# g8a9/multi-modal-emotion

Hardware: AMD Instinct MI355X
Metric: utterances/sec fwd+bwd (+clip_grad_norm_+AdamW inside the timed step), TAV (BERT+Wav2Vec2+VideoMAE) b=32, 1/2/4/8 MI355X (higher is better)
Workload: dtype bf16; 1 GPU; tav_nn.py TAV preset B (bert 12 L + wav2vec2 12 L / 768 + videomae 12 L / 768 on 16 frames + fusion 12 L), global batch 32 = 32 per GPU x 1, text 128 tok, audio 80000 samples, video 16x3x224x224 (104 fusion / 1464 encoder tokens), 547.0 GFLOP forward per utterance; global_batch=32, per_gpu_batch=32, parallelism=dp1, weights=random init (seeded), no checkpoints offline, launch=hipGraph replay

## Files before the change

### include/tavhip.h

```cpp
#ifndef TAVHIP_H
#define TAVHIP_H
#include <stdint.h>

#ifdef __cplusplus
extern "C" {
#endif

enum { TAV_F32 = 0, TAV_BF16 = 1, TAV_FP8 = 2 ,
       TAV_U8 = 3 ,
       TAV_I16 = 4  };
enum {
    TAV_ERR_NULL = -1,
    TAV_ERR_SHAPE = -2,
    TAV_ERR_DTYPE = -3,
    TAV_ERR_ALIGN = -4,
    TAV_ERR_NO_RCCL = -5
};

int tav_version(void);
const char* tav_error_string(int code);

typedef struct tav_gemm_nt_args {
    const void* A; const void* B; void* C;
    void* C_pre;
// ... 15 lines not shown
} tav_gemm_nt_args;
int tav_gemm_nt(const tav_gemm_nt_args* args, void* stream);
int tav_gemm_nt_schedule(const tav_gemm_nt_args* args, int32_t* tile, int32_t* rows_first, int32_t* tile_rest);

typedef struct tav_gemm_tn_args {
    const void* A; const void* B;
    float* slabs;
    float* out;
    float* dbias;
    float* bias_partials;
    int64_t N1, N2;
    int64_t lda, ldb;
    int64_t rows_per_batch, nbatch;
    int64_t a_zb, b_zb;
    int32_t chunk_rows, nsplit;
    int32_t perm_inner, perm_outer;
    int32_t dtype;
    int32_t accumulate;
    float scale;
} tav_gemm_tn_args;
int tav_gemm_tn_splits(int64_t n1, int64_t n2, int64_t rows_per_batch, int64_t nbatch, int32_t* chunk_rows, int32_t* nsplit);
int tav_gemm_tn(const tav_gemm_tn_args* args, void* stream);

typedef struct tav_gemm_tn_problem {
    const void* A; const void* B;
    float* out;
    float* dbias;
    int64_t N1, N2, lda, ldb;
} tav_gemm_tn_problem;
int tav_gemm_tn_grouped(const tav_gemm_tn_problem* problems, int32_t nproblems, int64_t rows, int32_t dtype, void* stream);
int64_t tav_gemm_tn_grouped_ws_bytes(const tav_gemm_tn_problem* problems, int32_t nproblems, int64_t rows, int32_t dtype, int32_t flags);
int tav_gemm_tn_grouped_ws(const tav_gemm_tn_problem* problems, int32_t nproblems, int64_t rows, int32_t dtype, void* workspace,
                           int64_t workspace_bytes, int32_t flags, void* stream);

int tav_fp8_amax_partials(int64_t rows, int64_t cols);
int tav_fp8_amax(const void* x, int32_t dtype, int64_t rows, int64_t cols, int64_t ld, float* partials, float* scales, void* stream);
int tav_fp8_quantize(const void* x, int32_t dtype, int64_t rows, int64_t cols, int64_t ld, const float* scales, void* q, int64_t ld_q, void* qt,
                     int64_t ld_qt, int64_t rows_pad, void* stream);
int tav_fp8_quantize_delayed(const void* x, int32_t dtype, int64_t rows, int64_t cols, int64_t ld, float* state, void* q, int64_t ld_q, void* qt,
                             int64_t ld_qt, int64_t rows_pad, void* stream);
int tav_fp8_roll_states(float* states, int64_t n, void* stream);
int tav_splitk_reduce(const float* slabs, float* out, int32_t nsplit, int64_t n_elems, int32_t accumulate, void* stream);

int tav_colsum(const void* x, int32_t dtype, int64_t M, int64_t N, int64_t ld, float* partials, int32_t nparts, float* out,
               int32_t accumulate, void* stream);

typedef struct tav_attn_args {
    const void* q; const void* k; const void* v;
    void* o;
    const float* key_mask;
    float* lse;
    float* corr;
    void* o_soft;
    const void* dout; void* dq; void* dk; void* dv;
    float* delta;
    int64_t B, S, nheads;
    int64_t ld_q, ld_k, ld_v, ld_o, ld_do, ld_dq, ld_dk, ld_dv;
    int32_t dtype, mask_mode;
    float scale;
    int32_t q_prescaled;
} tav_attn_args;
int tav_attn_fwd(const tav_attn_args* args, void* stream);
int tav_attn_bwd(const tav_attn_args* args, void* stream);
int tav_attn_fwd_len(const tav_attn_args* args, const int32_t* seq_lens, void* stream);
int tav_attn_bwd_len(const tav_attn_args* args, const int32_t* seq_lens, void* stream);
int tav_attn_probs(const tav_attn_args* args, float* probs, const float* head_scale, int64_t hs_bstride, void* stream);
// ... 190 lines not shown
```

### multi-modal-emotion_amd/_lib.py

```python
import ctypes as C
import os

import torch

_HERE = os.path.dirname(os.path.abspath(__file__))
LIB_PATH = os.environ.get("TAV_LIB") or os.path.join(_HERE, "libtavhip.so")

TAV_F32, TAV_BF16, TAV_FP8, TAV_U8, TAV_I16 = 0, 1, 2, 3, 4
ABI_VERSION = 7

i32, i64, f32, vp = C.c_int32, C.c_int64, C.c_float, C.c_void_p


class GemmNTArgs(C.Structure):
    _fields_ = [("A", vp), ("B", vp), ("C", vp), ("C_pre", vp), ("bias", vp), ("gelu_in", vp), ("resid", vp),
                ("M", i64), ("N", i64), ("K", i64),
                ("lda", i64), ("ldb", i64), ("ldc", i64), ("ld_pre", i64), ("ld_gelu_in", i64), ("ld_resid", i64),
                ("nzb", i32), ("nzg", i32),
                ("a_zb", i64), ("a_zg", i64), ("b_zb", i64), ("b_zg", i64), ("c_zb", i64), ("c_zg", i64), ("bias_zg", i64),
                ("in_dtype", i32), ("out_dtype", i32), ("act", i32), ("accumulate", i32), ("alpha", f32),
                ("a_dequant", vp), ("b_dequant", vp), ("gelu_zb", i64), ("tile_m_hint", i32)]


class GemmTNArgs(C.Structure):
    _fields_ = [("A", vp), ("B", vp), ("slabs", vp), ("out", vp), ("dbias", vp), ("bias_partials", vp),
                ("N1", i64), ("N2", i64), ("lda", i64), ("ldb", i64), ("rows_per_batch", i64), ("nbatch", i64),
                ("a_zb", i64), ("b_zb", i64), ("chunk_rows", i32), ("nsplit", i32), ("perm_inner", i32), ("perm_outer", i32),
                ("dtype", i32), ("accumulate", i32), ("scale", f32)]


class GemmTNProblem(C.Structure):
    _fields_ = [("A", vp), ("B", vp), ("out", vp), ("dbias", vp), ("N1", i64), ("N2", i64), ("lda", i64), ("ldb", i64)]


class AttnArgs(C.Structure):
    _fields_ = [("q", vp), ("k", vp), ("v", vp), ("o", vp), ("key_mask", vp), ("lse", vp), ("corr", vp), ("o_soft", vp),
                ("dout", vp), ("dq", vp), ("dk", vp), ("dv", vp), ("delta", vp),
                ("B", i64), ("S", i64), ("nheads", i64),
                ("ld_q", i64), ("ld_k", i64), ("ld_v", i64), ("ld_o", i64), ("ld_do", i64), ("ld_dq", i64), ("ld_dk", i64), ("ld_dv", i64),
                ("dtype", i32), ("mask_mode", i32), ("scale", f32), ("q_prescaled", i32)]


class LnArgs(C.Structure):
    _fields_ = [("x", vp), ("x_dtype", i32), ("gamma", vp), ("beta", vp), ("y_f32", vp), ("y_lp", vp), ("lp_dtype", i32),
                ("mean", vp), ("rstd", vp),
                ("dy", vp), ("dy_dtype", i32), ("dx_add", vp), ("dx_f32", vp), ("dx_lp", vp),
                ("dgamma", vp), ("dbeta", vp), ("partials", vp), ("accumulate_params", i32),
                ("rows", i64), ("W", i64), ("ld_x", i64), ("ld_y", i64), ("ld_dy", i64), ("ld_dx", i64), ("eps", f32), ("act", i32),
                ("defer_param_reduce", i32)]


class LnReduceItem(C.Structure):
    _fields_ = [("partials", vp), ("dgamma", vp), ("dbeta", vp), ("nblocks", i32), ("W", i32), ("accumulate", i32), ("pad_", i32)]


LN_REDUCE_MAX = 64


class TextEmbedArgs(C.Structure):
    _fields_ = [("ids", vp), ("word", vp), ("pos", vp), ("type", vp), ("gamma", vp), ("beta", vp), ("pre", vp), ("pos_ids", vp),
                ("y_f32", vp), ("y_lp", vp), ("lp_dtype", i32), ("mean", vp), ("rstd", vp),
                ("B", i64), ("S", i64), ("W", i64), ("vocab", i64), ("max_pos", i64), ("pad_id", i32), ("eps", f32)]


class ClipXform(C.Structure):
    _fields_ = [("src_dtype", i32), ("T", i32), ("H", i32), ("W", i32), ("sT", i64), ("sH", i64), ("sW", i64), ("sC", i64),
                ("nf", i32), ("frame", i32 * 32), ("crop_top", i32), ("crop_left", i32), ("crop_h", i32), ("crop_w", i32),
                ("mid_h", i32), ("mid_w", i32), ("out_h", i32), ("out_w", i32), ("hflip", i32), ("vflip", i32),
                ("scale", f32 * 3), ("shift", f32 * 3)]


class ResampleArgs(C.Structure):
    _fields_ = [("src_dtype", i32), ("C", i32), ("L", i64), ("sC", i64), ("sL", i64), ("o", i32), ("n", i32), ("width", i32), ("ntap", i32),
                ("first_max", i32), ("reserved", i32), ("T_row", i64)]


_SIGS = {
    "tav_version": (C.c_int, []),
    "tav_error_string": (C.c_char_p, [C.c_int]),
    "tav_gemm_nt": (C.c_int, [C.POINTER(GemmNTArgs), vp]),
    "tav_gemm_nt_schedule": (C.c_int, [C.POINTER(GemmNTArgs), C.POINTER(i32), C.POINTER(i32), C.POINTER(i32)]),
    "tav_gemm_tn_splits": (C.c_int, [i64, i64, i64, i64, C.POINTER(i32), C.POINTER(i32)]),
    "tav_gemm_tn": (C.c_int, [C.POINTER(GemmTNArgs), vp]),
    "tav_gemm_tn_grouped": (C.c_int, [C.POINTER(GemmTNProblem), i32, i64, i32, vp]),
    "tav_gemm_tn_grouped_ws_bytes": (C.c_int64, [C.POINTER(GemmTNProblem), i32, i64, i32, i32]),
    "tav_gemm_tn_grouped_ws": (C.c_int, [C.POINTER(GemmTNProblem), i32, i64, i32, vp, i64, i32, vp]),
    "tav_colsum": (C.c_int, [vp, i32, i64, i64, i64, vp, i32, vp, i32, vp]),
    "tav_fp8_amax_partials": (C.c_int, [i64, i64]),
    "tav_fp8_amax": (C.c_int, [vp, i32, i64, i64, i64, vp, vp, vp]),
    "tav_fp8_quantize": (C.c_int, [vp, i32, i64, i64, i64, vp, vp, i64, vp, i64, i64, vp]),
    "tav_fp8_quantize_delayed": (C.c_int, [vp, i32, i64, i64, i64, vp, vp, i64, vp, i64, i64, vp]),
    "tav_fp8_roll_states": (C.c_int, [vp, i64, vp]),
    "tav_splitk_reduce": (C.c_int, [vp, vp, i32, i64, i32, vp]),
    "tav_comm_rccl_version": (C.c_int, [C.POINTER(i32)]),
    "tav_comm_unique_id": (C.c_int, [vp]),
    "tav_comm_init_rank": (C.c_int, [C.POINTER(vp), i32, vp, i32]),
    "tav_comm_destroy": (C.c_int, [vp]),
    "tav_allreduce_bucket": (C.c_int, [vp, i64, i32, vp, vp]),
    "tav_attn_fwd": (C.c_int, [C.POINTER(AttnArgs), vp]),
    "tav_attn_bwd": (C.c_int, [C.POINTER(AttnArgs), vp]),
    "tav_attn_fwd_len": (C.c_int, [C.POINTER(AttnArgs), vp, vp]),
    "tav_attn_bwd_len": (C.c_int, [C.POINTER(AttnArgs), vp, vp]),
    "tav_attn_probs": (C.c_int, [C.POINTER(AttnArgs), vp, vp, i64, vp]),
    "tav_head_scale": (C.c_int, [vp, vp, vp, i32, vp, i64, f32, i64, i64, i64, i64, i64, i64, vp]),
    "tav_ln_fwd": (C.c_int, [C.POINTER(LnArgs), vp]),
    "tav_ln_bwd": (C.c_int, [C.POINTER(LnArgs), vp]),
    "tav_ln_bwd_partials": (C.c_int, [i64]),
    "tav_ln_param_reduce_multi": (C.c_int, [C.POINTER(LnReduceItem), i32, vp]),
    "tav_cast_weight": (C.c_int, [vp, i64, i64, vp, i64, vp, i64, i32, vp]),
    "tav_cast_weights_multi": (C.c_int, [vp, i32, i32, vp]),
    "tav_cast_conv_weight": (C.c_int, [vp, i64, i64, i64, vp, vp, vp, i64, i32, vp]),
    "tav_zero_pad_rows": (C.c_int, [vp, i32, i64, i64, i64, i64, vp]),
    "tav_cast2d": (C.c_int, [vp, i32, i64, vp, i32, i64, i64, i64, vp]),
    "tav_transpose2d": (C.c_int, [vp, vp, i32, i64, i64, i64, vp]),
    "tav_add_f32": (C.c_int, [vp, vp, vp, vp, i32, i64, vp]),
    "tav_fill_f32": (C.c_int, [vp, f32, i64, vp]),
    "tav_embed_add_fwd": (C.c_int, [vp, vp, vp, vp, i64, i64, i64, vp]),
    "tav_embed_add_bwd": (C.c_int, [vp, vp, vp, vp, i64, i64, i64, i32, vp]),
    "tav_embed_add_bwd_parts": (C.c_int, [i64]),
# ... 100 lines not shown
```

### multi-modal-emotion_amd/csrc/gemm.hip

```cpp
#include "common.h"
#include <type_traits>
#include "tavhip_internal.h"
#include "gemm_plan.h"

namespace tav {

struct GemmNT {
    const char* A; const char* B; char* C; char* Cpre; const float* bias; const char* gelu_in; const float* resid;
    int M, N, K;
    long lda, ldb, ldc, ld_pre, ld_gelu, ld_resid;
    int nzg;
    long a_zb, a_zg, b_zb, b_zg, c_zb, c_zg, bias_zg;
    long g_zb;
    int act, accumulate;
    float alpha;
    int tiles_m, tiles_n;
    const float* sa; const float* sb;
};

TAV_DEV int swz(int row, int chunk) { return chunk ^ ((row >> 1) & 7); }

enum { NT_GEN = 0, NT_PLAIN = 1, NT_RESID = 2, NT_GELU_D = 3, NT_MUL_D = 4 };
template <typename T, typename TO, int TM, int NST, int NW, int TNW, int EPI = NT_GEN>
__global__ __launch_bounds__(64 * NW, NW == 4 ? 2 : 1) __attribute__((amdgpu_waves_per_eu(2, 2))) void gemm_nt_kernel(const GemmNT p) {
// ... 503 lines not shown
    for (int a = 0; a < 4; ++a) {
        const int n1 = n1_0 + w1 * 64 + a * 16 + i;
        if (n1 >= p.N1) continue;
#pragma unroll
        for (int b = 0; b < 4; ++b) {
            const int n2 = n2_0 + w2 * 64 + b * 16 + 4 * g;
            if (n2 >= p.N2) continue;
            st4(S + (long)n1 * p.N2 + n2, acc[a][b]);
        }
    }
}

template <typename T>
__global__ __launch_bounds__(256, 2) void gemm_tn_kernel(const GemmTN p) {
    gemm_tn_body<T>(p, xcd_remap(blockIdx.x, p.tiles_1 * p.tiles_2), blockIdx.y);
}

constexpr int TN_GROUP_MAX = 4;
struct GemmTNGroup {
    GemmTN p[TN_GROUP_MAX];
    int tile_end[TN_GROUP_MAX];
    int n;
};
template <typename T>
__global__ __launch_bounds__(256, 2) void gemm_tn_grouped_kernel(const GemmTNGroup grp) {
    const int t = xcd_remap(blockIdx.x, grp.tile_end[grp.n - 1]);
    int g = 0;
#pragma unroll
    for (int k = 0; k < TN_GROUP_MAX - 1; ++k) g += (k < grp.n - 1 && t >= grp.tile_end[k]) ? 1 : 0;
    const int first = g == 0 ? 0 : grp.tile_end[g - 1];
    gemm_tn_body<T>(grp.p[g], t - first, 0);
}

template <typename T>
TAV_DEV void gemm_tn_big_body(const GemmTN& p, const int tile, const int split) {
    using TT = TNTile<T>;
    static_assert(ET<T>::ES == 2, "bf16 only");
    constexpr int ES = 2, KSTEP = ET<T>::KSTEP, KT = 64, ROWB = TT::ROWB;
    constexpr int SUB = KT * ROWB;
    constexpr int STAGE = 4 * SUB;
    extern __shared__ __attribute__((aligned(16))) char smem[];

    const int tid = threadIdx.x, lane = tid & 63, wave = tid >> 6;
    const int g = lane >> 4, i = lane & 15;
    const int w1 = wave >> 1, w2 = wave & 1;

    int t1, t2;
    if (p.tiles_1 >= p.tiles_2) { t1 = tile / p.tiles_2; t2 = tile - t1 * p.tiles_2; }
    else { t2 = tile / p.tiles_1; t1 = tile - t2 * p.tiles_1; }
    const int n1_0 = t1 * 256, n2_0 = t2 * 256;
    const int row_begin = split * p.chunk_rows;
    int row_end = row_begin + p.chunk_rows; row_end = row_end < p.rows_per_batch ? row_end : p.rows_per_batch;
    const int nrows = row_end - row_begin;
    const int nk = nrows > 0 ? (nrows + KT - 1) / KT : 0;

    const int lrow = lane >> 4, lslot = lane & 15;
    const int a_cmax = (p.N1 - n1_0) * ES / 16, b_cmax = (p.N2 - n2_0) * ES / 16;
    const char* Ab0 = p.A + ((long)row_begin * p.lda + n1_0) * ES;
    const char* Bb0 = p.B + ((long)row_begin * p.ldb + n2_0) * ES;
    unsigned offA[2][2], offB[2][2];
#pragma unroll
    for (int h = 0; h < 2; ++h)
#pragma unroll
        for (int j = 0; j < 2; ++j) {
            const int trow = wave * 8 + j * 4 + lrow;
            int ca = 16 * h + TT::sw(trow, lslot); ca = ca < a_cmax ? ca : 0;
// ... 129 lines not shown
    long end4[TN_GROUP_MAX];
    int N1[TN_GROUP_MAX];
    int nbias[TN_GROUP_MAX];
    int n, nsplit;
};
__global__ void tn_group_reduce_kernel(const TNGroupReduce r) {
    const long gid = (long)blockIdx.x * blockDim.x + threadIdx.x;
    if (gid >= r.end4[r.n - 1]) return;
    int k = 0;
#pragma unroll
    for (int q = 0; q < TN_GROUP_MAX - 1; ++q) k += (q < r.n - 1 && gid >= r.end4[q]) ? 1 : 0;
    const long local = gid - (k == 0 ? 0 : r.end4[k - 1]);
    const float* S = r.slabs[k];
    f32x4 v = {0.f, 0.f, 0.f, 0.f};
    for (int s2 = 0; s2 < r.nsplit; ++s2) v += ld4(S + ((long)s2 * r.n4[k] + local) * 4);
    st4(r.out[k] + local * 4, v);
    if (r.dbias[k] && local < r.N1[k]) {
        float b = 0.f;
        for (int s2 = 0; s2 < r.nbias[k]; ++s2) b += r.bias_part[k][(long)s2 * r.N1[k] + local];
        r.dbias[k][local] = b;
    }
}
__global__ void tn_group_bias_reduce_kernel(const TNGroupReduce r, int total_n1) {
    int gid = blockIdx.x * blockDim.x + threadIdx.x;
    if (gid >= total_n1) return;
    int k = 0;
    while (k < r.n - 1 && gid >= r.N1[k]) { gid -= r.N1[k]; ++k; }
    if (!r.dbias[k]) return;
    float b = 0.f;
    for (int s2 = 0; s2 < r.nbias[k]; ++s2) b += r.bias_part[k][(long)s2 * r.N1[k] + gid];
    r.dbias[k][gid] = b;
}

__global__ void splitk_reduce_kernel(const float* __restrict__ S, float* __restrict__ out, int nsplit, long n_elems, int N2,
                                     int inner, int outer, int accumulate, float scale, const float* __restrict__ bias_part,
                                     float* __restrict__ dbias, int N1) {
    const long gid = (long)blockIdx.x * blockDim.x + threadIdx.x;
    if (dbias && gid < N1) {
        float b = 0.f;
        for (int s = 0; s < nsplit; ++s) b += bias_part[(long)s * N1 + gid];
        b *= scale;
        dbias[gid] = accumulate ? dbias[gid] + b : b;
    }
    const long idx4 = gid * 4;
    if (idx4 >= n_elems) return;
    f32x4 v = {0.f, 0.f, 0.f, 0.f};
    for (int s = 0; s < nsplit; ++s) v += ld4(S + (long)s * n_elems + idx4);
    v *= scale;
    if (outer == 1) {
        if (accumulate) v += ld4(out + idx4);
        st4(out + idx4, v);
    } else {
        const long n1 = idx4 / N2; const int n2 = (int)(idx4 - n1 * N2);
#pragma unroll
        for (int e = 0; e < 4; ++e) {
            const int q = n2 + e;
            const long o = n1 * N2 + (long)(q % inner) * outer + q / inner;
            out[o] = accumulate ? out[o] + v[e] : v[e];
        }
    }
}

__global__ void bias_reduce_kernel(const float* __restrict__ part, float* __restrict__ out, int nsplit, int N1, int accumulate, float scale) {
    const int n = blockIdx.x * blockDim.x + threadIdx.x;
    if (n >= N1) return;
    float s = 0.f;
    for (int k = 0; k < nsplit; ++k) s += part[(long)k * N1 + n];
    s *= scale;
    out[n] = accumulate ? out[n] + s : s;
}

template <typename T>
__global__ void colsum_partial_kernel(const T* __restrict__ X, float* __restrict__ part, int M, int N, long ld, int rows_per_block) {
    const int n = blockIdx.x * blockDim.x + threadIdx.x;
    const int r_begin = blockIdx.y * rows_per_block;
    int r_end = r_begin + rows_per_block; r_end = r_end < M ? r_end : M;
    if (n >= N) return;
    float s0 = 0.f, s1 = 0.f, s2 = 0.f, s3 = 0.f;
    int r = r_begin;
    for (; r + 3 < r_end; r += 4) {
        s0 += ET<T>::ld(X + (long)r * ld + n); s1 += ET<T>::ld(X + (long)(r + 1) * ld + n);
        s2 += ET<T>::ld(X + (long)(r + 2) * ld + n); s3 += ET<T>::ld(X + (long)(r + 3) * ld + n);
    }
    for (; r < r_end; ++r) s0 += ET<T>::ld(X + (long)r * ld + n);
    part[(long)blockIdx.y * N + n] = (s0 + s1) + (s2 + s3);
}
__global__ void colsum_final_kernel(const float* __restrict__ part, float* __restrict__ out, int nparts, int N, int accumulate) {
    const int n = blockIdx.x * blockDim.x + threadIdx.x;
    if (n >= N) return;
    float s0 = 0.f, s1 = 0.f, s2 = 0.f, s3 = 0.f;
    int k = 0;
    for (; k + 3 < nparts; k += 4) {
        s0 += part[(long)k * N + n]; s1 += part[(long)(k + 1) * N + n]; s2 += part[(long)(k + 2) * N + n]; s3 += part[(long)(k + 3) * N + n];
// ... 147 lines not shown
    { const int rc = plan::tn_validate_problem(a->A, a->B, a->out, a->N1, a->N2, a->lda, a->ldb, a->a_zb, a->b_zb, a->rows_per_batch, a->nbatch, a->dtype);
      if (rc != 0) return rc; }
    if (a->chunk_rows <= 0 || a->chunk_rows % 64) return TAV_ERR_SHAPE;
    GemmTN p;
    p.A = (const char*)a->A; p.B = (const char*)a->B; p.S = a->slabs;
    p.bias_part = a->dbias ? a->bias_partials : nullptr; p.bias_spread = 0;
    if (a->dbias && !a->bias_partials) return TAV_ERR_NULL;
    p.N1 = (int)a->N1; p.N2 = (int)a->N2; p.lda = a->lda; p.ldb = a->ldb;
    p.rows_per_batch = (int)a->rows_per_batch; p.a_zb = a->a_zb; p.b_zb = a->b_zb;
    p.chunk_rows = a->chunk_rows;
    p.chunks_per_batch = (int)((a->rows_per_batch + a->chunk_rows - 1) / a->chunk_rows);
    const int nsplit = p.chunks_per_batch * (int)a->nbatch;
    if (nsplit != a->nsplit) return TAV_ERR_SHAPE;
    p.tiles_1 = (p.N1 + 127) / 128; p.tiles_2 = (p.N2 + 127) / 128;
    const int inner = a->perm_inner > 0 ? a->perm_inner : p.N2, outer = a->perm_outer > 0 ? a->perm_outer : 1;
    if (outer > 1 && inner * outer != p.N2) return TAV_ERR_SHAPE;
    dim3 grid(p.tiles_1 * p.tiles_2, nsplit), block(256);
    if (a->dtype == TAV_BF16) {
        const size_t lds = 4 * 64 * 256;
        hipLaunchKernelGGL((gemm_tn_kernel<bf16>), grid, block, lds, stream, p);
    } else {
        const size_t lds = 4 * 64 * 512;
        hipLaunchKernelGGL((gemm_tn_kernel<float>), grid, block, lds, stream, p);
    }
    int e = (int)hipGetLastError();
    if (e) return e;
    const long n_elems = (long)p.N1 * p.N2;
    const long nthreads = (n_elems + 3) / 4;
    hipLaunchKernelGGL(splitk_reduce_kernel, dim3((unsigned)((nthreads + 255) / 256)), dim3(256), 0, stream, a->slabs, a->out, nsplit,
                       n_elems, p.N2, inner, outer, a->accumulate, a->scale == 0.f ? 1.f : a->scale, (const float*)a->bias_partials, a->dbias, p.N1);
    return (int)hipGetLastError();
}

extern "C" int tav_colsum(const void* x, int32_t dtype, int64_t M, int64_t N, int64_t ld, float* partials, int32_t nparts, float* out,
                          int32_t accumulate, void* stream_) {
    hipStream_t stream = (hipStream_t)stream_;
    if (!x || !partials || !out) return TAV_ERR_NULL;
    if (M <= 0 || N <= 0 || nparts <= 0) return TAV_ERR_SHAPE;
    const int rows_per_block = (int)((M + nparts - 1) / nparts);
    dim3 grid((unsigned)((N + 255) / 256), nparts), block(256);
    if (dtype == TAV_BF16) hipLaunchKernelGGL((colsum_partial_kernel<bf16>), grid, block, 0, stream, (const bf16*)x, partials, (int)M, (int)N, (long)ld, rows_per_block);
    else if (dtype == TAV_F32) hipLaunchKernelGGL((colsum_partial_kernel<float>), grid, block, 0, stream, (const float*)x, partials, (int)M, (int)N, (long)ld, rows_per_block);
    else return TAV_ERR_DTYPE;
    hipLaunchKernelGGL(colsum_final_kernel, dim3((unsigned)((N + 255) / 256)), dim3(256), 0, stream, partials, out, nparts, (int)N, accumulate);
    return (int)hipGetLastError();
}
```

### multi-modal-emotion_amd/csrc/gemm_plan.h

```cpp
#pragma once
#include <stdint.h>
#include <algorithm>
#include "../../include/tavhip.h"

namespace tav {
namespace plan {

inline int elem_size(int dtype) { return dtype == TAV_FP8 ? 1 : (dtype == TAV_BF16 ? 2 : 4); }

inline int nt_validate(const tav_gemm_nt_args* a, bool need_ptrs) {
    if (!a || (need_ptrs && (!a->A || !a->B || !a->C))) return TAV_ERR_NULL;
    if (a->M <= 0 || a->N <= 0 || a->K <= 0) return TAV_ERR_SHAPE;
    const int es = elem_size(a->in_dtype);
    if (a->in_dtype != TAV_BF16 && a->in_dtype != TAV_F32 && a->in_dtype != TAV_FP8) return TAV_ERR_DTYPE;
    if (a->in_dtype == TAV_F32 && a->out_dtype != TAV_F32) return TAV_ERR_DTYPE;
    if (a->out_dtype != TAV_F32 && a->out_dtype != TAV_BF16) return TAV_ERR_DTYPE;
    if ((a->K * es) % 128 != 0) return TAV_ERR_SHAPE;
    if ((a->M * a->lda + a->K) * es >= (1ll << 32) || (a->N * a->ldb + a->K) * es >= (1ll << 32)) return TAV_ERR_SHAPE;
    if (a->N % 4 != 0) return TAV_ERR_SHAPE;
    {
        const int64_t ldmax = std::max(std::max(a->ldc, a->C_pre ? a->ld_pre : 0), std::max(a->gelu_in ? a->ld_gelu_in : 0, a->resid ? a->ld_resid : 0));
        if (ldmax < 0 || 256 * ldmax + a->N >= (1ll << 30)) return TAV_ERR_SHAPE;
    }
    const int pk = 16 / es;
// ... 150 lines not shown
    if ((rows_per_batch + 64) * (lda > ldb ? lda : ldb) * es >= (1ll << 32)) return TAV_ERR_SHAPE;
    return 0;
}
inline int tn_validate_group(const tav_gemm_tn_problem* probs, int nprob, int64_t rows, int dtype) {
    for (int k = 0; k < nprob; ++k) {
        const tav_gemm_tn_problem& a = probs[k];
        const int rc = tn_validate_problem(a.A, a.B, a.out, a.N1, a.N2, a.lda, a.ldb, 0, 0, rows, 1, dtype);
        if (rc != 0) return rc;
    }
    return 0;
}

constexpr double TN_SPLIT_PENALTY = 0.06;
inline void tn_splits(int64_t n1, int64_t n2, int64_t rows_per_batch, int64_t nbatch, int32_t* chunk_rows, int32_t* nsplit) {
    const long tiles = ((n1 + 127) / 128) * ((n2 + 127) / 128);
    const long SLOTS = 512;
    long best_cpb = 1, best_cr = ((rows_per_batch + 63) / 64) * 64; double best_score = -1.0;
    const long max_cpb = (rows_per_batch + 255) / 256 > 0 ? (rows_per_batch + 255) / 256 : 1;
    for (long cpb = 1; cpb <= max_cpb && cpb <= 64; ++cpb) {
        long cr = (rows_per_batch + cpb - 1) / cpb;
        cr = ((cr + 63) / 64) * 64;
        const long real_cpb = (rows_per_batch + cr - 1) / cr;
        const long wgs = tiles * real_cpb * nbatch;
        const long rounds = (wgs + SLOTS - 1) / SLOTS;
        const double work = (double)rounds * (double)cr;
        const double ideal = (double)tiles * nbatch * rows_per_batch / SLOTS;
        const double score = ideal / work - TN_SPLIT_PENALTY * (double)(real_cpb * nbatch);
        if (score > best_score + 1e-9) { best_score = score; best_cpb = real_cpb; best_cr = cr; }
    }
    *chunk_rows = (int32_t)best_cr;
    *nsplit = (int32_t)(best_cpb * nbatch);
}

struct TnGroupPlan {
    bool big;
    int tw, nsplit;
    long chunk;
    long ws_floats;
};
inline TnGroupPlan tn_big_plan(const tav_gemm_tn_problem* probs, int nprob, long rows, int dtype, int flags) {
    TnGroupPlan P{false, 128, 1, 0, 0};
    const bool can_big = dtype == TAV_BF16 && !(flags & 2);
    long tiles = 0, elems = 0;
    for (int k = 0; k < nprob; ++k) {
        tiles += ((probs[k].N1 + 255) / 256) * ((probs[k].N2 + 255) / 256);
        elems += probs[k].N1 * probs[k].N2;
    }
    P.big = can_big && ((flags & 1) || (rows >= 12288 && tiles >= 48));
    if (P.big) {
        int best = 1; double best_score = -1.0;
        for (int s2 = 1; s2 <= 4; ++s2) {
            if (s2 > 1 && rows / s2 < 2048) break;
            const long wgs = tiles * s2;
            const double fill = (double)wgs / (double)(((wgs + 255) / 256) * 256);
            const double score = fill - 0.04 * (s2 - 1);
            if (score > best_score + 1e-9) { best_score = score; best = s2; }
        }
        if ((flags >> 8) & 15) best = (flags >> 8) & 15;
        P.nsplit = best;
        P.tw = 256;
    }
    P.chunk = ((rows + P.nsplit - 1) / P.nsplit + 63) / 64 * 64;
    P.ws_floats = P.nsplit > 1 ? (long)P.nsplit * elems : 0;
    for (int k = 0; k < nprob; ++k)
        if (probs[k].dbias) P.ws_floats += (long)P.nsplit * ((probs[k].N2 + P.tw - 1) / P.tw) * probs[k].N1;
    return P;
// ... 45 lines not shown
```

### multi-modal-emotion_amd/engine.py

```python
import weakref

import torch

from . import ops

_EPOCH = [0]


def bump_weight_epoch():
    _EPOCH[0] += 1


class Policy:

    def __init__(self, name="bf16", fp8_fwd=None, fp8_bwd=None):
        name = {"bfloat16": "bf16", "float32": "fp32", "f32": "fp32", "float8": "fp8", "e4m3": "fp8"}.get(name, name)
        if name not in ("bf16", "fp32", "fp8", "fp8-all", "fp8-wgrad8"):
            raise ValueError(f"unknown precision policy {name!r}")
        self.name = name
        self.lp = torch.float32 if name == "fp32" else torch.bfloat16
        self.f32 = name == "fp32"
        self.fp8 = name.startswith("fp8")
        self.fp8_stacks = () if not self.fp8 else (("video", "text", "audio", "fusion") if name == "fp8-all" else ("video",))
        self.fp8_wgrad8 = name in ("fp8-wgrad8", "fp8-all")
# ... 602 lines not shown
        if ctx.has_b and ctx.needs_input_grad[3]:
            db = ops.colsum(du_pad.view(B * TP, Co) if du_pad is not None else du.view(B * T_out, Co))
        if want_dx and phase:
            if ctx.chained:
                out = ops.zero_pad_rows(torch.empty(B, T_in + 2 * P, Ci, dtype=du_v.dtype, device=du_v.device), B, T_in, Ci, P)
                zc, obase = (T_in + 2 * P) * Ci, P * Ci
            else:
                out = torch.empty(B, T_in, Ci, dtype=du_v.dtype, device=du_v.device)
                zc, obase = T_in * Ci, 0
            oflat, aflat, uflat = out.view(-1), du_pad.view(-1), (u_in.reshape(-1) if ctx.chained else None)
            off = 0
            for r in range(stride):
                Q = (k - r + stride - 1) // stride
                Mr = (T_in - r + stride - 1) // stride
                ops.gemm_nt(aflat[(P - (Q - 1)) * Co:], w_ph[off:off + Ci * Q * Co], out=oflat[obase + r * Ci:], M=Mr, N=Ci, K=Q * Co, lda=Co, ldb=Q * Co,
                            ldc=stride * Ci, nzb=B, a_zb=TP * Co, c_zb=zc, gelu_in=uflat[r * Ci:] if ctx.chained else None,
                            ld_gelu=stride * Ci, gelu_zb=T_in * Ci)
                off += Ci * Q * Co
            if ctx.chained:
                dui = out[:, P:P + T_in]
                _CONV_PADDED[dui.data_ptr()] = out
            else:
                dx = out
        elif want_dx:
            dcol = ops.gemm_nt(_c(du_v).view(B * T_out, Co), w_t, out_shape=(B * T_out, k * Ci))
            d = ops.col2im_1d(dcol, B, T_in, T_out, Ci, k, stride, pre_act=u_in if ctx.chained else None)
            if ctx.chained:
                dui = d
            else:
                dx = d
        return dx, dui, dw, db, None, None, None


class PosConvFn(torch.autograd.Function):

    @staticmethod
    def forward(ctx, x, v, g, bias, B, T, G, ectx):
        pol = ectx.pol
        x = _c(x)
        H = x.shape[1]
        Cg, K = H // G, v.shape[2]
        w, _, norms = ectx.cache.posconv(v, g)
        pad = K // 2
        xg = ops.group_pad(x, B, T, H, G, pad, pad, pol.lp)
        TP = T + 2 * pad
        y, pre = ops.gemm_nt(xg, w, bias=bias, act=1, resid=x, want_pre=True, out_dtype=torch.float32, M=T, N=Cg, K=K * Cg, lda=Cg, ldb=K * Cg,
                             ldc=H, nzb=B, nzg=G, a_zb=G * TP * Cg, a_zg=TP * Cg, b_zg=Cg * K * Cg, c_zb=T * H, c_zg=Cg, bias_zg=Cg,
                             out_shape=(B * T, H))
        ctx.ectx, ctx.geom = ectx, (B, T, H, G, Cg, K)
        ctx.save_for_backward(xg, pre, v, g, norms)
        return y

    @staticmethod
    def backward(ctx, gout):
        xg, pre, v, g, norms = ctx.saved_tensors
        pol = ctx.ectx.pol
        B, T, H, G, Cg, K = ctx.geom
        gout = _c(gout)
        _, wf, _ = ctx.ectx.cache.posconv(v, g)
        du = ops.gelu_bwd(pre, gout)
        pad = K // 2
        dug = ops.group_pad(du, B, T, H, G, pad - 1, pad, pol.lp)
        TPd, TP = T + 2 * pad - 1, T + 2 * pad
        dx = ops.gemm_nt(dug, wf, resid=gout, out_dtype=torch.float32, M=T, N=Cg, K=K * Cg, lda=Cg, ldb=K * Cg, ldc=H, nzb=B, nzg=G,
                         a_zb=G * TPd * Cg, a_zg=TPd * Cg, b_zg=Cg * K * Cg, c_zb=T * H, c_zg=Cg, out_shape=(B * T, H))
        du_lp = _to_lp(pol, du)
        dw = torch.empty(G, Cg, K * Cg, dtype=torch.float32, device=du.device)
        for gi in range(G):
            ops.gemm_tn(du_lp[:, gi * Cg:], xg[:, gi], out=dw[gi], N1=Cg, N2=K * Cg, lda=H, ldb=Cg, rows_per_batch=T, nbatch=B, a_zb=T * H,
                        b_zb=G * TP * Cg)
        dv, dg = ops.weight_norm_bwd(v, g, norms, dw)
        dbias = ops.colsum(du)
        return dx, dv, dg.view_as(g), dbias, None, None, None, None


class ConcatSeqFn(torch.autograd.Function):

    @staticmethod
    def forward(ctx, B, *parts):
        W = parts[0].shape[-1]
        lens = [p.numel() // (B * W) for p in parts]
        Sf = sum(lens)
        out = torch.empty(B, Sf, W, dtype=torch.float32, device=parts[0].device)
        flat = out.view(B, Sf * W)
        off = 0
        for p, L in zip(parts, lens):
            ops.cast2d(_c(p).view(B, L * W), torch.float32, out=flat[:, off * W:(off + L) * W])
            off += L
        ctx.lens, ctx.W, ctx.B = lens, W, B
        return out

    @staticmethod
    def backward(ctx, g):
        B, W = ctx.B, ctx.W
        flat = _c(g).view(B, -1)
        outs, off = [], 0
        for L in ctx.lens:
            outs.append(ops.cast2d(flat[:, off * W:(off + L) * W], torch.float32).view(B * L, W))
            off += L
        return (None, *outs)


class TailFn(torch.autograd.Function):
# ... 204 lines not shown
```

### multi-modal-emotion_amd/ops.py

```python
import ctypes as C
import math

import numpy as np
import torch

from . import _lib as L
from ._lib import check, dt, lib, ptr, stream

_ws = {}


def workspace(name, nfloats, device):
    key = (name, torch.cuda.current_stream().cuda_stream, str(device))
    t = _ws.get(key)
    if t is None or t.numel() < nfloats:
        t = torch.empty(max(int(nfloats), 1), dtype=torch.float32, device=device)
        _ws[key] = t
    return t


def clear_workspaces():
    _ws.clear()


# ... 76 lines not shown
    _prof_launch("gemm_nt", sel, 2.0 * M * N * K * nz, nbytes, lambda: check(lib().tav_gemm_nt(C.byref(g), stream()), "gemm_nt"))
    return (out, pre) if want_pre else out


def gemm_tn(a, b, *, out=None, accumulate=False, N1=None, N2=None, lda=None, ldb=None, rows_per_batch=None, nbatch=1,
            a_zb=0, b_zb=0, perm_inner=0, perm_outer=0, scale=1.0, out_shape=None, want_bias=False):
    if N1 is None:
        N1, N2 = a.shape[-1], b.shape[-1]
        rows_per_batch = a.shape[-2]
        lda, ldb = a.stride(-2), b.stride(-2)
    cr, ns = C.c_int32(), C.c_int32()
    check(lib().tav_gemm_tn_splits(N1, N2, rows_per_batch, nbatch, C.byref(cr), C.byref(ns)), "gemm_tn_splits")
    slabs = workspace("tn_slabs", ns.value * N1 * N2, a.device)
    if out is None:
        out = torch.empty(out_shape or (N1, N2), dtype=torch.float32, device=a.device)
    g = L.GemmTNArgs()
    g.A, g.B, g.slabs, g.out = ptr(a), ptr(b), ptr(slabs), ptr(out)
    g.N1, g.N2, g.lda, g.ldb = N1, N2, lda, ldb
    g.rows_per_batch, g.nbatch, g.a_zb, g.b_zb = rows_per_batch, nbatch, a_zb, b_zb
    g.chunk_rows, g.nsplit, g.perm_inner, g.perm_outer = cr.value, ns.value, perm_inner, perm_outer
    g.dtype, g.accumulate, g.scale = dt(a), int(accumulate), scale
    dbias = None
    if want_bias:
        dbias = torch.empty(N1, dtype=torch.float32, device=a.device)
        bpart = workspace("tn_bias", ns.value * N1, a.device)
        g.dbias, g.bias_partials = ptr(dbias), ptr(bpart)
    assert a.dtype == b.dtype
    tokens = rows_per_batch * nbatch
    _prof_launch("gemm_tn", "bf16" if a.dtype == torch.bfloat16 else "f32", 2.0 * tokens * N1 * N2, tokens * (N1 + N2) * a.element_size() + 4 * N1 * N2,
                 lambda: check(lib().tav_gemm_tn(C.byref(g), stream()), "gemm_tn"))
    return (out, dbias) if want_bias else out


def gemm_tn_grouped(pairs, want_bias=True, flags=0, into=None):
    n = len(pairs)
    rows, dtype = pairs[0][0].shape[0], pairs[0][0].dtype
    probs = (L.GemmTNProblem * n)()
    outs = []
    for k, (a, b) in enumerate(pairs):
        assert a.shape[0] == rows and b.shape[0] == rows and a.dtype == dtype and b.dtype == dtype
        N1, N2 = a.shape[1], b.shape[1]
        dW_to, db_to = into[k] if into is not None else (None, None)
        dW = dW_to if dW_to is not None else torch.empty(N1, N2, dtype=torch.float32, device=a.device)
        db = (db_to if db_to is not None else torch.empty(N1, dtype=torch.float32, device=a.device)) if want_bias else None
        assert dW.shape == (N1, N2) and dW.is_contiguous() and dW.dtype == torch.float32 and (db is None or (db.shape == (N1,) and db.is_contiguous()))
        pr = probs[k]
        pr.A, pr.B, pr.out, pr.dbias = ptr(a), ptr(b), ptr(dW), ptr(db)
        pr.N1, pr.N2, pr.lda, pr.ldb = N1, N2, a.stride(0), b.stride(0)
        outs.append((dW, db))
    nbytes = lib().tav_gemm_tn_grouped_ws_bytes(probs, n, rows, dt(pairs[0][0]), flags)
    ws = torch.empty(nbytes, dtype=torch.uint8, device=pairs[0][0].device) if nbytes > 0 else None
    es = pairs[0][0].element_size()
    _prof_launch("gemm_tn", "bf16" if dtype == torch.bfloat16 else "f32", sum(2.0 * rows * a.shape[1] * b.shape[1] for a, b in pairs),
                 sum(rows * (a.shape[1] + b.shape[1]) * es + 4 * a.shape[1] * b.shape[1] for a, b in pairs),
                 lambda: check(lib().tav_gemm_tn_grouped_ws(probs, n, rows, dt(pairs[0][0]), ptr(ws), nbytes, flags, stream()), "gemm_tn_grouped"))
    return outs


FP8 = torch.float8_e4m3fn
FP8_KPAD = 1024


class Fp8:
    __slots__ = ("q", "qt", "scales", "rows", "cols")

    def __init__(self, q, qt, scales, rows, cols):
# ... 855 lines not shown
```

Measured before the change: 428.8 utterances/s.

## Batch wav2vec2 positional-conv weight-grad GEMMs across groups in one launch

Replaces the per-group loop of gemm_tn calls in the positional-conv backward with a single batched TN GEMM kernel that puts groups on the grid z dimension and splits batches across grid y. A reduce kernel then sums the split slabs per group. It also reads the already padded low-precision gradient directly instead of casting du again, removing one conversion pass and G-1 launch and reduce pairs. The cost is a new kernel with its own split planner and a larger slab workspace, and correctness depends on the offset view into dug lining up with the earlier layout.

```diff
diff --git a/include/tavhip.h b/include/tavhip.h
--- a/include/tavhip.h
+++ b/include/tavhip.h
@@ -71,6 +71,25 @@
 int64_t tav_gemm_tn_grouped_ws_bytes(const tav_gemm_tn_problem* problems, int32_t nproblems, int64_t rows, int32_t dtype, int32_t flags);
 int tav_gemm_tn_grouped_ws(const tav_gemm_tn_problem* problems, int32_t nproblems, int64_t rows, int32_t dtype, void* workspace,
                            int64_t workspace_bytes, int32_t flags, void* stream);
+
+typedef struct tav_gemm_tn_batched_args {
+    const void* A; const void* B;
+    float* slabs;
+    float* out;
+    int64_t N1, N2;
+    int64_t lda, ldb;
+    int64_t rows_per_batch, nbatch;
+    int64_t a_zb, b_zb;
+    int64_t a_zg, b_zg, out_zg;
+    int32_t ngroup, batches_per_split;
+    int32_t perm_inner, perm_outer;
+    int32_t dtype;
+    int32_t accumulate;
+    float scale;
+} tav_gemm_tn_batched_args;
+int tav_gemm_tn_batched_plan(int64_t n1, int64_t n2, int64_t rows_per_batch, int64_t nbatch, int64_t ngroup, int32_t* batches_per_split,
+                             int32_t* nsplit, int64_t* workspace_bytes);
+int tav_gemm_tn_batched(const tav_gemm_tn_batched_args* args, void* stream);
 
 int tav_fp8_amax_partials(int64_t rows, int64_t cols);
 int tav_fp8_amax(const void* x, int32_t dtype, int64_t rows, int64_t cols, int64_t ld, float* partials, float* scales, void* stream);
diff --git a/multi-modal-emotion_amd/_lib.py b/multi-modal-emotion_amd/_lib.py
--- a/multi-modal-emotion_amd/_lib.py
+++ b/multi-modal-emotion_amd/_lib.py
@@ -27,6 +27,13 @@
                 ("N1", i64), ("N2", i64), ("lda", i64), ("ldb", i64), ("rows_per_batch", i64), ("nbatch", i64),
                 ("a_zb", i64), ("b_zb", i64), ("chunk_rows", i32), ("nsplit", i32), ("perm_inner", i32), ("perm_outer", i32),
                 ("dtype", i32), ("accumulate", i32), ("scale", f32)]
+
+
+class GemmTNBatchedArgs(C.Structure):
+    _fields_ = [("A", vp), ("B", vp), ("slabs", vp), ("out", vp),
+                ("N1", i64), ("N2", i64), ("lda", i64), ("ldb", i64), ("rows_per_batch", i64), ("nbatch", i64),
+                ("a_zb", i64), ("b_zb", i64), ("a_zg", i64), ("b_zg", i64), ("out_zg", i64), ("ngroup", i32), ("batches_per_split", i32),
+                ("perm_inner", i32), ("perm_outer", i32), ("dtype", i32), ("accumulate", i32), ("scale", f32)]
 
 
 class GemmTNProblem(C.Structure):
@@ -85,6 +92,8 @@
     "tav_gemm_tn_grouped": (C.c_int, [C.POINTER(GemmTNProblem), i32, i64, i32, vp]),
     "tav_gemm_tn_grouped_ws_bytes": (C.c_int64, [C.POINTER(GemmTNProblem), i32, i64, i32, i32]),
     "tav_gemm_tn_grouped_ws": (C.c_int, [C.POINTER(GemmTNProblem), i32, i64, i32, vp, i64, i32, vp]),
+    "tav_gemm_tn_batched_plan": (C.c_int, [i64, i64, i64, i64, i64, C.POINTER(i32), C.POINTER(i32), C.POINTER(i64)]),
+    "tav_gemm_tn_batched": (C.c_int, [C.POINTER(GemmTNBatchedArgs), vp]),
     "tav_colsum": (C.c_int, [vp, i32, i64, i64, i64, vp, i32, vp, i32, vp]),
     "tav_fp8_amax_partials": (C.c_int, [i64, i64]),
     "tav_fp8_amax": (C.c_int, [vp, i32, i64, i64, i64, vp, vp, vp]),
diff --git a/multi-modal-emotion_amd/csrc/gemm.hip b/multi-modal-emotion_amd/csrc/gemm.hip
--- a/multi-modal-emotion_amd/csrc/gemm.hip
+++ b/multi-modal-emotion_amd/csrc/gemm.hip
@@ -559,6 +559,138 @@
     gemm_tn_body<T>(grp.p[g], t - first, 0);
 }
 
+struct GemmTNBatched {
+    const char* A; const char* B; float* S;
+    int N1, N2;
+    long lda, ldb;
+    int rows_per_batch, nbatch;
+    long a_zb, b_zb, a_zg, b_zg;
+    int bps, nsplit;
+    int tiles_1, tiles_2;
+};
+template <typename T>
+TAV_DEV void gemm_tn_batched_body(const GemmTNBatched& p, const int tile, const int split, const int group) {
+    using TT = TNTile<T>;
+    constexpr int ES = ET<T>::ES, KSTEP = ET<T>::KSTEP;
+    constexpr int BT = 128, KT = TNShape<T>::KT, NST = TNShape<T>::NST;
+    constexpr int ROWB = TT::ROWB, CPR = TT::CPR;
+    constexpr int TILE_BYTES = KT * ROWB;
+    constexpr int RPI = 64 / CPR, WROWS = KT / 4, NINST = WROWS / RPI;
+    static_assert(KT % KSTEP == 0 && WROWS % RPI == 0 && NINST >= 1, "TN tile shape");
+    static_assert(NST == 2, "the waits below are derived for a two-buffer ring");
+    extern __shared__ __attribute__((aligned(16))) char smem[];
+    char* sA = smem;
+    char* sB = smem + NST * TILE_BYTES;
+
+    const int tid = threadIdx.x, lane = tid & 63, wave = tid >> 6;
+    const int g = lane >> 4, i = lane & 15;
+    const int w1 = wave >> 1, w2 = wave & 1;
+    int t1, t2;
+    if (p.tiles_1 >= p.tiles_2) { t1 = tile / p.tiles_2; t2 = tile - t1 * p.tiles_2; }
+    else { t2 = tile / p.tiles_1; t1 = tile - t2 * p.tiles_1; }
+    const int n1_0 = t1 * BT, n2_0 = t2 * BT;
+    const int zb0 = split * p.bps;
+    const int nent = (zb0 + p.bps <= p.nbatch ? p.bps : p.nbatch - zb0);
+    const int nrows = p.rows_per_batch;
+    const int nk = (nrows + KT - 1) / KT;
+    const int nf = nent * nk;
+
+    const int lrow = lane / CPR, lslot = lane % CPR;
+    const int a_cmax = (p.N1 - n1_0) * ES / 16, b_cmax = (p.N2 - n2_0) * ES / 16;
+
+    f32x4 acc[4][4];
+#pragma unroll
+    for (int a = 0; a < 4; ++a)
+#pragma unroll
+        for (int b = 0; b < 4; ++b) acc[a][b] = f32x4{0.f, 0.f, 0.f, 0.f};
+
+    const unsigned ldsA = __builtin_amdgcn_readfirstlane(lds_addr(sA) + wave * WROWS * ROWB);
+    const unsigned ldsB = __builtin_amdgcn_readfirstlane(lds_addr(sB) + wave * WROWS * ROWB);
+    unsigned offA[NINST], offB[NINST];
+#pragma unroll
+    for (int j = 0; j < NINST; ++j) {
+        const int trow = wave * WROWS + j * RPI + lrow;
+        int ca = TT::sw(trow, lslot); ca = ca < a_cmax ? ca : 0;
+        int cb = TT::sw(trow, lslot); cb = cb < b_cmax ? cb : 0;
+        offA[j] = (unsigned)(trow * p.lda * ES + ca * 16);
+        offB[j] = (unsigned)(trow * p.ldb * ES + cb * 16);
+    }
+    const unsigned strideA = (unsigned)(KT * p.lda * ES), strideB = (unsigned)(KT * p.ldb * ES);
+    const long entA = p.a_zb * ES, entB = p.b_zb * ES;
+    const char* sAe = p.A + ((long)group * p.a_zg + (long)zb0 * p.a_zb + n1_0) * ES;
+    const char* sBe = p.B + ((long)group * p.b_zg + (long)zb0 * p.b_zb + n2_0) * ES;
+    int skt = 0;
+    auto stage_next = [&](int buf) {
+        const bool full = (skt + 1) * KT <= nrows;
+        if (full) {
+            const unsigned ka = skt * strideA, kb = skt * strideB;
+#pragma unroll
+            for (int j = 0; j < NINST; ++j) {
+                glds16_m0(sAe + ka, offA[j], ldsA + buf * TILE_BYTES + j * 1024);
+                glds16_m0(sBe + kb, offB[j], ldsB + buf * TILE_BYTES + j * 1024);
+            }
+        } else {
+#pragma unroll 1
+            for (int j = 0; j < NINST; ++j) {
+                const int trow = wave * WROWS + j * RPI + lrow;
+                const int ca = TT::sw(trow, lslot), cb = TT::sw(trow, lslot);
+                const long row = (long)skt * KT + trow;
+                const bool ok = row < nrows;
+                uint4 va = make_uint4(0, 0, 0, 0), vb = va;
+                if (ok && ca < a_cmax) va = *reinterpret_cast<const uint4*>(sAe + row * p.lda * ES + ca * 16);
+                if (ok && cb < b_cmax) vb = *reinterpret_cast<const uint4*>(sBe + row * p.ldb * ES + cb * 16);
+                *reinterpret_cast<uint4*>(sA + buf * TILE_BYTES + trow * ROWB + lslot * 16) = va;
+                *reinterpret_cast<uint4*>(sB + buf * TILE_BYTES + trow * ROWB + lslot * 16) = vb;
+            }
+        }
+        if (++skt == nk) { skt = 0; sAe += entA; sBe += entB; }
+    };
+    auto compute = [&](int cur) {
+        const char* cA = sA + cur * TILE_BYTES;
+        const char* cB = sB + cur * TILE_BYTES;
+#pragma unroll
+        for (int s = 0; s < KT / KSTEP; ++s) {
+            uint4 f1[4], f2[4];
+#pragma unroll
+            for (int t = 0; t < 4; ++t) {
+                f1[t] = tn_frag<T>(cA, s * KSTEP, w1 * 64 + t * 16, lane);
+                f2[t] = tn_frag<T>(cB, s * KSTEP, w2 * 64 + t * 16, lane);
+            }
+#pragma unroll
+            for (int a = 0; a < 4; ++a)
+#pragma unroll
+                for (int b = 0; b < 4; ++b) mma16<T>(f2[b], f1[a], acc[a][b]);
+        }
+    };
+
+    stage_next(0);
+    int cur = 0;
+    for (int f = 0; f < nf; ++f) {
+        wait_vmcnt0();
+        __syncthreads();
+        if (f + 1 < nf) stage_next(cur ^ 1);
+        compute(cur);
+        cur ^= 1;
+    }
+
+    float* S = p.S + ((long)group * p.nsplit + split) * p.N1 * p.N2;
+#pragma unroll
+    for (int a = 0; a < 4; ++a) {
+        const int n1 = n1_0 + w1 * 64 + a * 16 + i;
+        if (n1 >= p.N1) continue;
+#pragma unroll
+        for (int b = 0; b < 4; ++b) {
+            const int n2 = n2_0 + w2 * 64 + b * 16 + 4 * g;
+            if (n2 >= p.N2) continue;
+            st4(S + (long)n1 * p.N2 + n2, acc[a][b]);
+        }
+    }
+}
+template <typename T>
+__global__ __launch_bounds__(256, 2) void gemm_tn_batched_kernel(const GemmTNBatched p) {
+    gemm_tn_batched_body<T>(p, xcd_remap(blockIdx.x, p.tiles_1 * p.tiles_2), blockIdx.y, blockIdx.z);
+}
+
 template <typename T>
 TAV_DEV void gemm_tn_big_body(const GemmTN& p, const int tile, const int split) {
     using TT = TNTile<T>;
@@ -754,6 +886,25 @@
     r.dbias[k][gid] = b;
 }
 
+TAV_DEV void splitk_sum_store(const float* __restrict__ S, float* __restrict__ out, int nsplit, long n_elems, int N2, int inner, int outer,
+                              int accumulate, float scale, long idx4) {
+    if (idx4 >= n_elems) return;
+    f32x4 v = {0.f, 0.f, 0.f, 0.f};
+    for (int s = 0; s < nsplit; ++s) v += ld4(S + (long)s * n_elems + idx4);
+    v *= scale;
+    if (outer == 1) {
+        if (accumulate) v += ld4(out + idx4);
+        st4(out + idx4, v);
+    } else {
+        const long n1 = idx4 / N2; const int n2 = (int)(idx4 - n1 * N2);
+#pragma unroll
+        for (int e = 0; e < 4; ++e) {
+            const int q = n2 + e;
+            const long o = n1 * N2 + (long)(q % inner) * outer + q / inner;
+            out[o] = accumulate ? out[o] + v[e] : v[e];
+        }
+    }
+}
 __global__ void splitk_reduce_kernel(const float* __restrict__ S, float* __restrict__ out, int nsplit, long n_elems, int N2,
                                      int inner, int outer, int accumulate, float scale, const float* __restrict__ bias_part,
                                      float* __restrict__ dbias, int N1) {
@@ -764,23 +915,13 @@
         b *= scale;
         dbias[gid] = accumulate ? dbias[gid] + b : b;
     }
-    const long idx4 = gid * 4;
-    if (idx4 >= n_elems) return;
-    f32x4 v = {0.f, 0.f, 0.f, 0.f};
-    for (int s = 0; s < nsplit; ++s) v += ld4(S + (long)s * n_elems + idx4);
-    v *= scale;
-    if (outer == 1) {
-        if (accumulate) v += ld4(out + idx4);
-        st4(out + idx4, v);
-    } else {
-        const long n1 = idx4 / N2; const int n2 = (int)(idx4 - n1 * N2);
-#pragma unroll
-        for (int e = 0; e < 4; ++e) {
-            const int q = n2 + e;
-            const long o = n1 * N2 + (long)(q % inner) * outer + q / inner;
-            out[o] = accumulate ? out[o] + v[e] : v[e];
-        }
-    }
+    splitk_sum_store(S, out, nsplit, n_elems, N2, inner, outer, accumulate, scale, gid * 4);
+}
+__global__ void tn_batched_reduce_kernel(const float* __restrict__ S, float* __restrict__ out, int nsplit, long n_elems, int N2, int inner,
+                                         int outer, int accumulate, float scale, long out_zg) {
+    const long gid = (long)blockIdx.x * blockDim.x + threadIdx.x;
+    splitk_sum_store(S + (long)blockIdx.y * nsplit * n_elems, out + (long)blockIdx.y * out_zg, nsplit, n_elems, N2, inner, outer, accumulate,
+                     scale, gid * 4);
 }
 
 __global__ void bias_reduce_kernel(const float* __restrict__ part, float* __restrict__ out, int nsplit, int N1, int accumulate, float scale) {
@@ -994,6 +1135,43 @@
     return (int)hipGetLastError();
 }
 
+extern "C" int tav_gemm_tn_batched_plan(int64_t n1, int64_t n2, int64_t rows_per_batch, int64_t nbatch, int64_t ngroup, int32_t* batches_per_split,
+                                        int32_t* nsplit, int64_t* workspace_bytes) {
+    if (!batches_per_split || !nsplit || !workspace_bytes) return TAV_ERR_NULL;
+    if (n1 <= 0 || n2 <= 0 || rows_per_batch <= 0 || nbatch <= 0 || ngroup <= 0) return TAV_ERR_SHAPE;
+    const plan::TnBatchedPlan P = plan::tn_batched_plan(n1, n2, rows_per_batch, nbatch, ngroup);
+    *batches_per_split = P.batches_per_split; *nsplit = P.nsplit; *workspace_bytes = P.ws_floats * 4;
+    return 0;
+}
+
+extern "C" int tav_gemm_tn_batched(const tav_gemm_tn_batched_args* a, void* stream_) {
+    hipStream_t stream = (hipStream_t)stream_;
+    if (!a || !a->slabs) return TAV_ERR_NULL;
+    { const int rc = plan::tn_validate_problem(a->A, a->B, a->out, a->N1, a->N2, a->lda, a->ldb, a->a_zb, a->b_zb, a->rows_per_batch, a->nbatch, a->dtype);
+      if (rc != 0) return rc; }
+    { const int rc = plan::tn_batched_validate(a->N1, a->N2, a->nbatch, a->ngroup, a->batches_per_split, a->a_zg, a->b_zg, a->out_zg, a->perm_inner,
+                                               a->perm_outer, a->dtype);
+      if (rc != 0) return rc; }
+    GemmTNBatched p;
+    p.A = (const char*)a->A; p.B = (const char*)a->B; p.S = a->slabs;
+    p.N1 = (int)a->N1; p.N2 = (int)a->N2; p.lda = a->lda; p.ldb = a->ldb;
+    p.rows_per_batch = (int)a->rows_per_batch; p.nbatch = (int)a->nbatch;
+    p.a_zb = a->a_zb; p.b_zb = a->b_zb; p.a_zg = a->a_zg; p.b_zg = a->b_zg;
+    p.bps = a->batches_per_split;
+    p.nsplit = (int)((a->nbatch + a->batches_per_split - 1) / a->batches_per_split);
+    p.tiles_1 = (p.N1 + 127) / 128; p.tiles_2 = (p.N2 + 127) / 128;
+    const int inner = a->perm_inner > 0 ? a->perm_inner : p.N2, outer = a->perm_outer > 0 ? a->perm_outer : 1;
+    dim3 grid(p.tiles_1 * p.tiles_2, p.nsplit, a->ngroup), block(256);
+    if (a->dtype == TAV_BF16) hipLaunchKernelGGL((gemm_tn_batched_kernel<bf16>), grid, block, 4 * 64 * 256, stream, p);
+    else hipLaunchKernelGGL((gemm_tn_batched_kernel<float>), grid, block, 4 * 64 * 512, stream, p);
+    int e = (int)hipGetLastError();
+    if (e) return e;
+    const long n_elems = (long)p.N1 * p.N2;
+    hipLaunchKernelGGL(tn_batched_reduce_kernel, dim3((unsigned)((n_elems / 4 + 255) / 256), a->ngroup), dim3(256), 0, stream, a->slabs, a->out,
+                       p.nsplit, n_elems, p.N2, inner, outer, a->accumulate, a->scale == 0.f ? 1.f : a->scale, (long)a->out_zg);
+    return (int)hipGetLastError();
+}
+
 extern "C" int tav_colsum(const void* x, int32_t dtype, int64_t M, int64_t N, int64_t ld, float* partials, int32_t nparts, float* out,
                           int32_t accumulate, void* stream_) {
     hipStream_t stream = (hipStream_t)stream_;
diff --git a/multi-modal-emotion_amd/csrc/gemm_plan.h b/multi-modal-emotion_amd/csrc/gemm_plan.h
--- a/multi-modal-emotion_amd/csrc/gemm_plan.h
+++ b/multi-modal-emotion_amd/csrc/gemm_plan.h
@@ -206,6 +206,35 @@
     *nsplit = (int32_t)(best_cpb * nbatch);
 }
 
+struct TnBatchedPlan {
+    int batches_per_split, nsplit;
+    long ws_floats;
+};
+constexpr long TN_BATCHED_FIXED_KT = 5;
+inline TnBatchedPlan tn_batched_plan(int64_t n1, int64_t n2, int64_t rows_per_batch, int64_t nbatch, int64_t ngroup) {
+    const long tiles = ((n1 + 127) / 128) * ((n2 + 127) / 128);
+    const long SLOTS = 512, nk = (rows_per_batch + 63) / 64;
+    long best_bps = nbatch, best_cost = -1;
+    for (long bps = nbatch; bps >= 1; --bps) {
+        const long ns = (nbatch + bps - 1) / bps;
+        if (bps > 1 && (nbatch + bps - 2) / (bps - 1) == ns) continue;
+        const long rounds = (tiles * ngroup * ns + SLOTS - 1) / SLOTS;
+        const long cost = rounds * (bps * nk + TN_BATCHED_FIXED_KT);
+        if (best_cost < 0 || cost < best_cost) { best_cost = cost; best_bps = bps; }
+    }
+    const long ns = (nbatch + best_bps - 1) / best_bps;
+    return TnBatchedPlan{(int)best_bps, (int)ns, ngroup * ns * n1 * n2};
+}
+inline int tn_batched_validate(int64_t N1, int64_t N2, int64_t nbatch, int64_t ngroup, int64_t batches_per_split, int64_t a_zg, int64_t b_zg,
+                               int64_t out_zg, int perm_inner, int perm_outer, int dtype) {
+    if (ngroup < 1 || ngroup > 65535 || batches_per_split < 1) return TAV_ERR_SHAPE;
+    if ((nbatch + batches_per_split - 1) / batches_per_split > 65535) return TAV_ERR_SHAPE;
+    const int pk = 16 / elem_size(dtype);
+    if (a_zg % pk || b_zg % pk || out_zg % 4) return TAV_ERR_ALIGN;
+    if (perm_outer > 1 && (int64_t)(perm_inner > 0 ? perm_inner : N2) * perm_outer != N2) return TAV_ERR_SHAPE;
+    return 0;
+}
+
 struct TnGroupPlan {
     bool big;
     int tw, nsplit;
diff --git a/multi-modal-emotion_amd/engine.py b/multi-modal-emotion_amd/engine.py
--- a/multi-modal-emotion_amd/engine.py
+++ b/multi-modal-emotion_amd/engine.py
@@ -658,6 +658,9 @@
         return dx, dui, dw, db, None, None, None
 
 
+_POSCONV_WGRAD_LOOP = False
+
+
 class PosConvFn(torch.autograd.Function):
 
     @staticmethod
@@ -690,11 +693,15 @@
         TPd, TP = T + 2 * pad - 1, T + 2 * pad
         dx = ops.gemm_nt(dug, wf, resid=gout, out_dtype=torch.float32, M=T, N=Cg, K=K * Cg, lda=Cg, ldb=K * Cg, ldc=H, nzb=B, nzg=G,
                          a_zb=G * TPd * Cg, a_zg=TPd * Cg, b_zg=Cg * K * Cg, c_zb=T * H, c_zg=Cg, out_shape=(B * T, H))
-        du_lp = _to_lp(pol, du)
         dw = torch.empty(G, Cg, K * Cg, dtype=torch.float32, device=du.device)
-        for gi in range(G):
-            ops.gemm_tn(du_lp[:, gi * Cg:], xg[:, gi], out=dw[gi], N1=Cg, N2=K * Cg, lda=H, ldb=Cg, rows_per_batch=T, nbatch=B, a_zb=T * H,
-                        b_zb=G * TP * Cg)
+        if _POSCONV_WGRAD_LOOP:
+            du_lp = _to_lp(pol, du)
+            for gi in range(G):
+                ops.gemm_tn(du_lp[:, gi * Cg:], xg[:, gi], out=dw[gi], N1=Cg, N2=K * Cg, lda=H, ldb=Cg, rows_per_batch=T, nbatch=B, a_zb=T * H,
+                            b_zb=G * TP * Cg)
+        else:
+            ops.gemm_tn_batched(dug.view(-1)[(pad - 1) * Cg:], xg, dw, N1=Cg, N2=K * Cg, lda=Cg, ldb=Cg, rows_per_batch=T, nbatch=B,
+                                a_zb=G * TPd * Cg, b_zb=G * TP * Cg, ngroup=G, a_zg=TPd * Cg, b_zg=TP * Cg, out_zg=Cg * K * Cg)
         dv, dg = ops.weight_norm_bwd(v, g, norms, dw)
         dbias = ops.colsum(du)
         return dx, dv, dg.view_as(g), dbias, None, None, None, None
diff --git a/multi-modal-emotion_amd/ops.py b/multi-modal-emotion_amd/ops.py
--- a/multi-modal-emotion_amd/ops.py
+++ b/multi-modal-emotion_amd/ops.py
@@ -132,6 +132,28 @@
     return (out, dbias) if want_bias else out
 
 
+def gemm_tn_batched(a, b, out, *, N1, N2, lda, ldb, rows_per_batch, nbatch, a_zb, b_zb, ngroup, a_zg, b_zg, out_zg, batches_per_split=0,
+                    perm_inner=0, perm_outer=0, scale=1.0, accumulate=False):
+    bps, ns, nbytes = C.c_int32(), C.c_int32(), C.c_int64()
+    check(lib().tav_gemm_tn_batched_plan(N1, N2, rows_per_batch, nbatch, ngroup, C.byref(bps), C.byref(ns), C.byref(nbytes)), "gemm_tn_batched_plan")
+    if batches_per_split > 0:
+        bps.value, ns.value = batches_per_split, -(-nbatch // batches_per_split)
+    slabs = workspace("tn_slabs", ngroup * ns.value * N1 * N2, a.device)
+    g = L.GemmTNBatchedArgs()
+    g.A, g.B, g.slabs, g.out = ptr(a), ptr(b), ptr(slabs), ptr(out)
+    g.N1, g.N2, g.lda, g.ldb = N1, N2, lda, ldb
+    g.rows_per_batch, g.nbatch, g.a_zb, g.b_zb = rows_per_batch, nbatch, a_zb, b_zb
+    g.a_zg, g.b_zg, g.out_zg, g.ngroup, g.batches_per_split = a_zg, b_zg, out_zg, ngroup, bps.value
+    g.perm_inner, g.perm_outer = perm_inner, perm_outer
+    g.dtype, g.accumulate, g.scale = dt(a), int(accumulate), scale
+    assert a.dtype == b.dtype and out.dtype == torch.float32
+    tokens = rows_per_batch * nbatch
+    _prof_launch("gemm_tn", "bf16" if a.dtype == torch.bfloat16 else "f32", 2.0 * tokens * N1 * N2 * ngroup,
+                 ngroup * (tokens * (N1 + N2) * a.element_size() + 4 * N1 * N2),
+                 lambda: check(lib().tav_gemm_tn_batched(C.byref(g), stream()), "gemm_tn_batched"))
+    return out
+
+
 def gemm_tn_grouped(pairs, want_bias=True, flags=0, into=None):
     n = len(pairs)
     rows, dtype = pairs[0][0].shape[0], pairs[0][0].dtype
```

New measurement: 430.6 utterances/s, median of 6. No clear change (+0.4%).
